# ksadov/FREUD

Hardware: AMD Instinct MI355X
Metric: SAE train activations/sec (d=384 dict 8x) (higher is better)
Workload: dtype bf16; 1 GPU; Whisper-tiny d=384 dict 8x (n=3072) L1 SAE train step, M=65536 rows/GPU/step, RAdam+cosine, x bfloat16 resident in HBM (BASELINE configs[1]); rows_per_gpu=65536, d_model=384, n_dict=3072, parallelism=dp1, dp=none

## Files before the change

freud_amd/csrc/bwd_fused.h:

```cpp
#pragma once
#include "common.h"
#include "gemm.h"

constexpr int BF_D = 384;
constexpr int BF_BM = 32;
constexpr int BF_BN = 128;
constexpr int BF_DXH_BYTES = BF_BM * BF_D * 2;
constexpr int BF_C_BYTES = BF_BM * BF_BN * 2;
constexpr int BF_STAGE_BYTES = 2 * BF_DXH_BYTES + BF_C_BYTES;
constexpr int BF_LDS_BYTES = 2 * BF_STAGE_BYTES;

__device__ __forceinline__ int dual_off(int row, int ch) {
  return row * 256 + ((ch ^ (((row & 3) << 2) | ((row >> 2) & 3))) << 4);
}

struct BwdFusedArgs {
  const bf16_t* dxh;
  const bf16_t* xb;
  const bf16_t* c;
  const bf16_t* Wt;
  const float* scal;
  int unscaled;
  const float* cnt_part;
  int n_cnt;
  float alpha;
  int64_t M;
  int d;
  float* slab;
  float* db_part;
  int n_p;
  int ntiles;
  int tile0;
  int splits;
  int steps_total;
  int bal_m, bal_q;
  const short* wg_map;
  unsigned long long* clk;
};

__device__ __forceinline__ bf16x8 tr_frag_perm(const char* img, int col0, int s, int lane) {
  const int h = lane >> 5, g = (lane >> 4) & 1, q = (lane & 15) >> 2, p = lane & 3;
  const int col = col0 + 16 * g + 4 * p;
  const int r0 = 16 * s + 4 * h + q, r1 = r0 + 8;
  const int o0 = dual_off(r0, col >> 3) + (col & 7) * 2;
  const int o1 = dual_off(r1, col >> 3) + (col & 7) * 2;
  const s16x4 lo = __builtin_amdgcn_ds_read_tr16_b64_v4i16(LDS_PTR(s16x4, img + o0));
  const s16x4 hi = __builtin_amdgcn_ds_read_tr16_b64_v4i16(LDS_PTR(s16x4, img + o1));
  typedef __attribute__((ext_vector_type(8))) short s16x8;
  const s16x8 v = __builtin_shufflevector(lo, hi, 0, 1, 2, 3, 4, 5, 6, 7);
  return __builtin_bit_cast(bf16x8, v);
}

constexpr int BF_RING = 12;

__device__ __forceinline__ void glds16_x2_add(const void* sbase0, const void* sbase1, unsigned voff0, unsigned voff1, unsigned base,
                                              unsigned l0, unsigned l1) {
  asm volatile(
      "s_add_u32 m0, %4, %5\n\ts_nop 0\n\tglobal_load_lds_dwordx4 %2, %0\n\t"
      "s_add_u32 m0, %4, %6\n\ts_nop 0\n\tglobal_load_lds_dwordx4 %3, %1"
      :
      : "s"(sbase0), "s"(sbase1), "v"(voff0), "v"(voff1), "s"(base), "s"(l0), "s"(l1)
      : "memory", "m0", "scc");
}
__device__ __forceinline__ void glds16_add(const void* sbase, unsigned voff, unsigned base, unsigned l0) {
  asm volatile("s_add_u32 m0, %2, %3\n\ts_nop 0\n\tglobal_load_lds_dwordx4 %1, %0" : : "s"(sbase), "v"(voff), "s"(base), "s"(l0) : "memory", "m0", "scc");
}
__device__ __forceinline__ void glds16_add_nt(const void* sbase, unsigned voff, unsigned base, unsigned l0) {
  asm volatile("s_add_u32 m0, %2, %3\n\ts_nop 0\n\tglobal_load_lds_dwordx4 %1, %0 nt" : : "s"(sbase), "v"(voff), "s"(base), "s"(l0) : "memory", "m0", "scc");
}
__device__ __forceinline__ void glds16_x2_add_nt(const void* sbase0, const void* sbase1, unsigned voff0, unsigned voff1, unsigned base,
                                                 unsigned l0, unsigned l1) {
  asm volatile(
      "s_add_u32 m0, %4, %5\n\ts_nop 0\n\tglobal_load_lds_dwordx4 %2, %0 nt\n\t"
      "s_add_u32 m0, %4, %6\n\ts_nop 0\n\tglobal_load_lds_dwordx4 %3, %1 nt"
      :
      : "s"(sbase0), "s"(sbase1), "v"(voff0), "v"(voff1), "s"(base), "s"(l0), "s"(l1)
      : "memory", "m0", "scc");
}

__global__ __launch_bounds__(256, 1) void bwd_fused_d384_kernel(BwdFusedArgs a) {
  extern __shared__ __attribute__((aligned(16))) char smem[];
  const int t = threadIdx.x, lane = t & 63, w = t >> 6;
  int qa = 0, qe = 1, wgk = 0;
  unsigned long long clk_k0 = 0;
  if (a.clk) clk_k0 = __builtin_amdgcn_s_memtime();
  int wgk_raw = (int)blockIdx.x;
  if (a.bal_m > 0 && a.wg_map) wgk_raw = (int)a.wg_map[blockIdx.x];
  double cnt_m = 0;
  if (a.cnt_part) {
    for (int i0 = t; i0 < a.n_cnt; i0 += 1024) {
      float cv[4];
#pragma unroll
      for (int u = 0; u < 4; ++u) cv[u] = a.cnt_part[min(i0 + 256 * u, a.n_cnt - 1)];
#pragma unroll
      for (int u = 0; u < 4; ++u) cnt_m += i0 + 256 * u < a.n_cnt ? (double)cv[u] : 0.0;
    }
  }
  if (a.bal_m > 0) {
    wgk = __builtin_amdgcn_readfirstlane(wgk_raw);
    qa = wgk * a.bal_m;
    qe = qa + a.bal_m < 32 * a.ntiles ? qa + a.bal_m : 32 * a.ntiles;
  }
  int n0 = 0, nw = 0;
  float scal1, scal2;
  if (a.cnt_part) {
    double* redc = reinterpret_cast<double*>(smem + BF_DXH_BYTES);
    double m = wave_sum_d(cnt_m);
    if (lane == 0) redc[w] = m;
    __syncthreads();
    const double count = (double)a.M * a.d - ((redc[0] + redc[1]) + (redc[2] + redc[3]));
    scal1 = a.alpha / (float)count;
    scal2 = 1.0f / (float)a.M;
    __syncthreads();
  } else {
    scal1 = a.scal[1];
    scal2 = a.scal[2];
  }
  const float scale = a.unscaled ? scal1 : 1.0f;
  const float inv_m = a.unscaled ? scal2 / scal1 : scal2;

  const int srow = lane >> 4;
  const int pc = lane & 15;
  unsigned voff_d[6], voff_c[2];
  unsigned loff_d[6];
#pragma unroll
// ... 72 lines not shown
  constexpr int RING = BF_RING, DIST = RING - 1;
  static_assert(72 % RING == 0, "ring slots must be static across steps");
  auto load_frag_s = [&](auto stage_tag, int i) -> bf16x8 {
    constexpr int ST = decltype(stage_tag)::value;
    if (i < 24) {
      return *reinterpret_cast<const bf16x8*>(smem + ST * BF_DXH_BYTES + (i >> 3) * 8192 + roff[i & 7]);
    } else {
      const int tt = i < 48 ? i - 24 : i - 48, dt = tt >> 1, sk = tt & 1;
      const char* b = smem + ST * BF_DXH_BYTES + (dt >> 2) * 8192 + sk * 4096;
      return i < 48 ? tr_pair(b + toff[2 * (dt & 3)], b + toff[2 * (dt & 3) + 1]) : tr_pair(b + toffX[2 * (dt & 3)], b + toffX[2 * (dt & 3) + 1]);
    }
  };
  auto load_c_s = [&](auto stage_tag, int half) -> bf16x8 {
    constexpr int ST = decltype(stage_tag)::value;
    const char* b = smem + ST * BF_C_BYTES + half * 4096;
    return tr_pair(b + coffC0, b + coffC1);
  };
  f32x16 cinit;
#pragma unroll
  for (int r = 0; r < 16; ++r) cinit[r] = inv_m;

  unsigned long long clk_t0 = 0, clk_r0 = 0, clk_loop = 0, clk_real = 0, clk_steps = 0;
#pragma unroll 1
  for (bool first_seg = true; qa < qe; first_seg = false) {
  bf16x8 wfrag[24];
  f32x16 acc[12];
  float db_acc = 0.f;
  bf16x8 ring[RING], cf[2], pf[2];
  int ntile, step_begin, step_end, split;
  if (a.bal_m > 0) {
    const int j = qa >> 5, qb = qe < 32 * (j + 1) ? qe : 32 * (j + 1);
    ntile = a.tile0 + j;
    step_begin = (qa - 32 * j) * a.bal_q;
    step_end = (qb - 32 * j) * a.bal_q;
    if (step_begin > a.steps_total) step_begin = a.steps_total;
    if (step_end > a.steps_total) step_end = a.steps_total;
    split = wgk - bal_first_wg(j, a.bal_m);
    qa = qb;
  } else {
    const int nblk = a.ntiles * a.splits;
    const int id = xcd_remap(blockIdx.x, nblk);
    split = id / a.ntiles;
    ntile = a.tile0 + id - split * a.ntiles;
    step_begin = (int)((int64_t)a.steps_total * split / a.splits);
    step_end = (int)((int64_t)a.steps_total * (split + 1) / a.splits);
    qa = qe;
  }
  ntile = __builtin_amdgcn_readfirstlane(ntile); step_begin = __builtin_amdgcn_readfirstlane(step_begin);
  step_end = __builtin_amdgcn_readfirstlane(step_end); split = __builtin_amdgcn_readfirstlane(split);
  n0 = ntile * BF_BN;
  nw = n0 + 32 * w;
  if (!first_seg) {
    asm volatile("s_waitcnt vmcnt(0) lgkmcnt(0)" ::: "memory");
    __syncthreads();
  }
  {
    const bf16_t* wp = a.Wt + (int64_t)(nw + (lane & 31)) * BF_D + 8 * (lane >> 5);
#pragma unroll
    for (int kk = 0; kk < 24; ++kk) wfrag[kk] = *reinterpret_cast<const bf16x8*>(wp + 16 * kk);
  }
#pragma unroll
  for (int i = 0; i < 12; ++i)
#pragma unroll
    for (int r = 0; r < 16; ++r) acc[i][r] = 0.f;
  db_acc = 0.f;
  if (step_begin < step_end) {
    const int64_t r0 = (int64_t)step_begin * BF_BM;
#pragma unroll
    for (int p = 0; p < 7; ++p) dma_pair_at(p, a.dxh + r0 * BF_D, a.xb + r0 * BF_D, a.c + r0 * a.n_p + n0, 0);
// ... 105 lines not shown
```

freud_amd/csrc/common.h:

```cpp
#pragma once
#include <hip/hip_runtime.h>
#include <stdint.h>

typedef __bf16 bf16_t;
typedef __attribute__((ext_vector_type(8))) __bf16 bf16x8;
typedef __attribute__((ext_vector_type(4))) __bf16 bf16x4;
typedef __attribute__((ext_vector_type(2))) __bf16 bf16x2;
typedef __attribute__((ext_vector_type(4))) short s16x4;
typedef __attribute__((ext_vector_type(16))) float f32x16;
typedef __attribute__((ext_vector_type(4))) float f32x4;
typedef __attribute__((ext_vector_type(4))) unsigned int u32x4;

#define LDS_PTR(T, p) ((__attribute__((address_space(3))) T*)(p))

__device__ __forceinline__ float bf16_round(float v) { return (float)(bf16_t)v; }

__device__ __forceinline__ float wave_sum(float v) {
#pragma unroll
  for (int o = 32; o > 0; o >>= 1) v += __shfl_xor(v, o, 64);
  return v;
}
__device__ __forceinline__ double wave_sum_d(double v) {
#pragma unroll
  for (int o = 32; o > 0; o >>= 1) v += __shfl_xor(v, o, 64);
// ... 44 lines not shown
      :
      : "s"(sbase0), "s"(sbase1), "v"(voff0), "v"(voff1), "s"(dst0), "s"(dst1)
      : "memory", "m0");
}

__device__ __forceinline__ void glds4(const void* sbase, unsigned voff, unsigned dst) {
  asm volatile("s_mov_b32 m0, %2\n\ts_nop 0\n\tglobal_load_lds_dword %1, %0" : : "s"(sbase), "v"(voff), "s"(dst) : "memory", "m0");
}

__device__ __forceinline__ void glds16(const void* sbase, unsigned voff, unsigned dst) {
  asm volatile("s_mov_b32 m0, %2\n\ts_nop 0\n\tglobal_load_lds_dwordx4 %1, %0" : : "s"(sbase), "v"(voff), "s"(dst) : "memory", "m0");
}

#include <type_traits>
template <int B, int E, class F>
__device__ __forceinline__ void static_for(F&& f) {
  if constexpr (B < E) {
    f(std::integral_constant<int, B>{});
    static_for<B + 1, E>(f);
  }
}

static inline int64_t round_up(int64_t v, int64_t m) { return (v + m - 1) / m * m; }

__host__ __device__ __forceinline__ int bal_first_wg(int j, int m) { return (32 * j) / m; }
__host__ __device__ __forceinline__ int bal_pieces(int j, int m) { return (32 * j + 31) / m - (32 * j) / m + 1; }
```

freud_amd/csrc/engine.hip:

```cpp
#include <hip/hip_runtime.h>
#include <math.h>
#include <stdarg.h>
#include <stdio.h>
#include <string.h>

#include <algorithm>
#include <utility>
#include <vector>

#include "../../include/freud_sae.h"
#include "l1_kernels.h"
#include "gemm256.h"
#include "gemm256s.h"
#include "gemm256_fp8.h"
#include "l1_fp8.h"
#include "dp_kernels.h"
#include "p2p_exchange.h"
#include <rccl/rccl.h>
#include <mutex>
#include <unistd.h>

static thread_local bool g_force_gemm128 = false;
static thread_local bool g_no_stream = false;
static thread_local int g_device = 0;
#include "bwd_fused.h"
#include "fwd_fused.h"
#include "fwd_fused2.h"
#include "topk_kernels.h"
#include "topk_sparse.h"
#include "topk_aux.h"
#include "eval_fp32.h"
#include "search.h"
#include "file_top.h"
#include "stats.h"
#include "coact.h"
#include "labels.h"
#include "manip.h"
#include "dict_match.h"

constexpr int G2_PERSIST_STATIC = 512;

static thread_local char g_err[512] = "";
static int fail(int code, const char* fmt, ...) {
  va_list ap;
  va_start(ap, fmt);
  vsnprintf(g_err, sizeof(g_err), fmt, ap);
  va_end(ap);
  return code;
// ... 187 lines not shown
  int dist_error = 0;
  char dist_errmsg[256] = "";
  bool p2p = false;
  int p2p_rank = 0;
  float* p2p_G[P2P_MAX_WORLD] = {};
  bf16_t* p2p_Gb[P2P_MAX_WORLD] = {};
  double* p2p_stats[P2P_MAX_WORLD] = {};
  unsigned long long* p2p_sig[P2P_MAX_WORLD] = {};
  void* p2p_opened[4 * P2P_MAX_WORLD] = {};
  int p2p_nopened = 0;
  unsigned long long* sig = nullptr;
  unsigned int* p2p_status = nullptr;
  unsigned int* p2p_status_host = nullptr;
  unsigned int* p2p_status_hostdev = nullptr;
  int p2p_fault_kind = 0, p2p_fault_rank = -1;
  unsigned long long p2p_fault_after = 0;
  float* col_stage = nullptr;
  float* audit_dst = nullptr;
  bool finegrained = false;
  unsigned long long p2p_epoch[P2P_CHANNELS] = {};
  unsigned long long p2p_epoch_push = 0;
  unsigned long long p2p_timeout_ticks = 12000000000ull;
  bool gn_from_exchange = false;
  int bal_m = 0;
  int bal_grid = 0;
  short* bal_map = nullptr;
  int bwd_ranges = 1;
  bool stats_inline = true;
  bool no_stream = false;
  int eval_prec = 0;
  LastCall last_call = LAST_FWD_BF16;
  void* fs_slab = nullptr;
  int8_t* co_zt = nullptr;
  int8_t* lb_lt = nullptr;
  int lb_rows = 0;
  float* mn_w = nullptr;
  int64_t e32_rows = 0;
  float *e32_x = nullptr, *e32_pre = nullptr, *e32_sel = nullptr, *e32_xhat = nullptr;
  double* e32_part = nullptr;
  int* e32_colmax = nullptr;
  int64_t step = 0;
  int64_t last_M = 0, last_M_p = 0;
  int last_dtype = 0;
  int profile = 0;
  int64_t prof_tick = 0;
  int prof_period = 8;
  EvRing ev[KID_COUNT];
  bool ev_init = false;
};
// ... 50 lines not shown
  }
}

extern "C" const char* sae_last_error(void) { return g_err; }
extern "C" int sae_version(void) { return 1; }
extern "C" const char* sae_kernel_name(int id) { return (id >= 0 && id < KID_COUNT) ? kKernelNames[id] : nullptr; }
extern "C" int sae_dominant_kernel(sae_ctx* c) { return c ? dominant_kid(c) : KID_DW; }

static int choose_splits(int r128, int c128, int64_t ktiles) {
  const bool big = !g_force_gemm128 && r128 % 2 == 0 && c128 % 2 == 0;
  const int tiles = big ? (r128 / 2) * (c128 / 2) : r128 * c128, slots = big ? 256 : 512;
  int best = 1;
  double best_cost = 1e30;
  for (int sp = 1; sp <= 16; ++sp) {
    if (sp > 1 && ktiles / sp < 8) break;
    const int rounds = (tiles * sp + slots - 1) / slots;
    const double cost = (double)rounds / sp + 0.04 * sp;
    if (cost < best_cost - 1e-9) {
      best_cost = cost;
      best = sp;
    }
  }
  return best;
}

static int fused_bwd_splits(int ntiles, int steps, int cols) {
  const double slab_steps = (double)cols * BF_D * 8.0 / 4.0e12 / 1.43e-6;
  int best = 1;
  double best_cost = 1e300;
  for (int sp = 1; sp <= 64 && sp <= steps; ++sp) {
    const int rounds = (ntiles * sp + 255) / 256;
    const double cost = rounds * ((double)((steps + sp - 1) / sp) + 5.0) + sp * slab_steps;
    if (cost < best_cost - 1e-9) {
      best_cost = cost;
      best = sp;
    }
  }
  return best;
}

static hipError_t peer_visible_malloc(const sae_ctx* c, void** p, size_t bytes) {
  if (c->finegrained) return hipExtMallocWithFlags(p, bytes, hipDeviceMallocFinegrained);
  return hipMalloc(p, bytes);
}

static int create_events(sae_ctx* c) {
// ... 120 lines not shown
  HIP_TRY(hipDeviceSynchronize());
  return SAE_OK;
}

extern "C" void sae_destroy(sae_ctx* c) {
  if (!c) return;
  (void)hipSetDevice(c->cfg.device_id);
  void* ptrs[] = {c->P,    c->Mom,     c->Var,     c->G,       c->Wb,   c->Wt,      c->xb,    c->c, c->dxh, c->dxhT, c->xT,
                  c->dpre, c->slab,    c->db_part, c->l1_part, c->sq_part, c->scal, c->gn_part, c->masked, c->cn_part, c->cnt_part,
                  c->We_b, c->Wd_b, c->xs, c->pre, c->dense, c->aux_dense, c->de_b, c->dh_b, c->e, c->dh, c->e2_part,
                  c->a2_part, c->dbd_part, c->ds_part, c->tkf, c->top_idx, c->aux_idx, c->tk, c->tv_part, c->nfsf, c->dead, c->dbe_fx,
                  c->multi_dense, c->multi_idx, c->em, c->dm_b, c->m2_part, c->x8, c->c8, c->W8, c->W8t, c->scal8, c->x8_part, c->dxh8,
                  c->stats, c->stats_part, c->Gb, c->top_vals, c->aux_vals, c->multi_vals, c->tile_max, c->sel_flag, c->csc_counts, c->csc_block_off, c->csc_total, c->csc_start, c->csc_item_start,
                  c->csc_item_latent, c->csc_entries, c->csc_part, c->csc_pbe, c->tkd, c->dead_cols, c->vec_rank, c->vec_bits, c->Wdd_b,
                  c->aux_dbe_part, c->be_r, c->cnorm, c->dw_tail, c->csc_multi, c->fs_slab, c->co_zt, c->lb_lt, c->mn_w};
  for (void* p : ptrs)
    if (p) (void)hipFree(p);
  if (c->dead_hint) (void)hipHostFree(c->dead_hint);
  for (int i = 0; i < c->p2p_nopened; ++i) (void)hipIpcCloseMemHandle(c->p2p_opened[i]);
  if (c->sig) (void)hipFree(c->sig);
  if (c->p2p_status) (void)hipFree(c->p2p_status);
  if (c->p2p_status_host) (void)hipHostFree(c->p2p_status_host);
  if (c->col_stage) (void)hipFree(c->col_stage);
  if (c->bal_map) (void)hipFree(c->bal_map);
  for (void* p : {(void*)c->e32_x, (void*)c->e32_pre, (void*)c->e32_sel, (void*)c->e32_xhat, (void*)c->e32_part, (void*)c->e32_colmax})
    if (p) (void)hipFree(p);
  if (c->comm) (void)ncclCommDestroy(c->comm);
  if (c->comm_stream) (void)hipStreamDestroy(c->comm_stream);
  for (hipEvent_t e : {c->ev_x, c->ev_stats, c->ev_done})
    if (e) (void)hipEventDestroy(e);
  for (hipEvent_t e : c->ev_range)
    if (e) (void)hipEventDestroy(e);
  if (c->ev_init)
    for (auto& r : c->ev)
      for (int i = 0; i < EV_RING; ++i) {
        if (r.beg[i]) (void)hipEventDestroy(r.beg[i]);
        if (r.end[i]) (void)hipEventDestroy(r.end[i]);
      }
  delete c;
}

extern "C" int sae_create(const sae_config* cfg, sae_ctx** out) {
  if (!cfg || !out) return fail(SAE_ERR_INVALID, "null argument");
  *out = nullptr;
  if (cfg->variant != SAE_VARIANT_L1 && cfg->variant != SAE_VARIANT_TOPK)
    return fail(SAE_ERR_INVALID, "Invalid autoencoder variant: %d, must be 'l1' or 'topk'", cfg->variant);
  if (cfg->variant == SAE_VARIANT_TOPK && (cfg->k <= 0 || cfg->k > cfg->n_dict || cfg->k > 1024))
// ... 57 lines not shown
    gemm_tail_plan((c->d_p / 256) * (c->n_p / 256), (int)(2 * Mp / 64), c->dw_tail_tiles, c->dw_tail_pieces);
    if ((c->d_p / 256) * (c->n_p / 256) % 256 == 0) c->dw_tail_tiles = c->dw_tail_pieces = -1;
  }
  c->dw_chunk_splits = choose_splits(c->dw_chunk_rows / 128, c->n_p / 128, 2 * Mp / 64);
  if (c->d_p >= 1024 && c->n_p % 256 == 0)
    for (int q = 4; q >= 2; --q)
      if ((c->n_p / 256) % q == 0) {
        c->dw_col_chunks = q;
        break;
      }
  c->dw_col_splits = choose_splits(c->d_p / 128, c->n_p / 128 / c->dw_col_chunks, 2 * Mp / 64);
  c->use_fused_bwd = (c->d_p == BF_D) && cfg->force_generic != 1 && !c->fp8;
  c->use_fused_fwd = (c->d_p == FF_D) && cfg->force_generic != 1 && !c->fp8;
  if (const char* fv = getenv("FREUD_FWD")) c->fwd_variant = atoi(fv) == 1 ? 1 : 2;
  c->bwd_splits = fused_bwd_splits(c->n_p / BF_BN, (int)(Mp / BF_BM), c->n_p);
  c->bwd_range_splits = c->bwd_splits;
  for (int r = 2; r <= 4; ++r)
    if ((c->n_p / BF_BN) % r == 0) {
      const int sp = fused_bwd_splits(c->n_p / BF_BN / r, (int)(Mp / BF_BM), c->n_p / r);
      if (sp > c->bwd_range_splits) c->bwd_range_splits = sp;
    }
  int slab_splits = c->use_fused_bwd ? (c->bwd_range_splits > c->dw_splits ? c->bwd_range_splits : c->dw_splits) : c->dw_splits;
  if (c->use_fused_bwd && c->cfg.debug_flags != 83 && !getenv("FREUD_BWD_UNIFORM")) {
    const int ntiles = c->n_p / BF_BN, cus = 256;
    const int m = (32 * ntiles + cus - 1) / cus, grid = (32 * ntiles + m - 1) / m;
    int pmax = 1;
    for (int j = 0; j < ntiles; ++j) pmax = bal_pieces(j, m) > pmax ? bal_pieces(j, m) : pmax;
    const int steps = (int)(Mp / BF_BM), q = (steps + 31) / 32;
    const double slab_steps = (double)c->n_p * BF_D * 8.0 / 4.0e12 / 1.43e-6;
    const double cost_bal = (double)m * q + 5.0 + (32 % m ? 3.5 : 0.0) + (32.0 / m + (32 % m ? 1.0 : 0.0)) * slab_steps;
    const int sp = c->bwd_splits, rounds = (ntiles * sp + 255) / 256;
    const double cost_uni = rounds * ((double)((steps + sp - 1) / sp) + 5.0) + sp * slab_steps;
    if (cost_bal < cost_uni * 0.995 && pmax <= 64 && grid <= 4096) {
      c->bal_m = m;
      c->bal_grid = grid;
      if (pmax > slab_splits) slab_splits = pmax;
      std::vector<int> order(grid);
      for (int k = 0; k < grid; ++k) order[k] = k;
      std::stable_sort(order.begin(), order.end(), [m](int a_, int b_) { return (a_ * m) % 32 < (b_ * m) % 32; });
      std::vector<short> map(grid);
      int pos = 0;
      for (int x = 0; x < 8; ++x) {
        const int len = grid / 8 + (x < grid % 8 ? 1 : 0);
        for (int i = 0; i < len; ++i) map[8 * i + x] = (short)order[pos++];
      }
      hipError_t e_ = hipMalloc((void**)&c->bal_map, (size_t)grid * 2);
      if (e_ == hipSuccess) e_ = hipMemcpy(c->bal_map, map.data(), (size_t)grid * 2, hipMemcpyHostToDevice);
      if (e_ != hipSuccess) {
        int rc_ = fail(SAE_ERR_HIP, "balanced backward: workgroup table: %s", hipGetErrorString(e_));
        sae_destroy(c);
        return rc_;
      }
    }
  }
  {
    const int64_t need = (int64_t)(c->dw_chunk_splits > c->dw_col_splits ? c->dw_chunk_splits : c->dw_col_splits);
    if (need > slab_splits) slab_splits = (int)need;
  }
  const int64_t db_rows = (Mp / 128) > 64 ? (Mp / 128) : 64;

#define ALLOC(ptr, bytes)                                   \
  do {                                                      \
    hipError_t e_ = hipMalloc((void**)&(ptr), (bytes));     \
    if (e_ != hipSuccess) {                                 \
      int rc_ = fail(SAE_ERR_HIP, "hipMalloc(%lld bytes) for %s failed: %s", (long long)(bytes), #ptr, \
                     hipGetErrorString(e_));                \
      sae_destroy(c);                                       \
      return rc_;                                           \
    }                                                       \
  } while (0)
  ALLOC(c->P, c->nparams * 4);
  ALLOC(c->Mom, c->nparams * 4);
  ALLOC(c->Var, c->nparams * 4);
  if (c->finegrained) {
    hipError_t e_ = peer_visible_malloc(c, (void**)&c->G, (size_t)(c->nparams + SAE_NUM_METRICS) * 4);
    if (e_ == hipSuccess) e_ = peer_visible_malloc(c, (void**)&c->stats, (size_t)DP_STATS_HEAD * 8);
    if (e_ != hipSuccess) {
      int rc_ = fail(SAE_ERR_HIP, "fine-grained allocation of the gradient / statistics buffers failed: %s", hipGetErrorString(e_));
      sae_destroy(c);
      return rc_;
    }
  } else {
// ... 1009 lines not shown
  if (rc) return rc;
  const bool fold_finalize = c->use_fused_fwd && c->use_fused_bwd && backward && gs == nullptr && c->bwd_ranges == 1 &&
                             c->cfg.debug_flags != 78;
  if (c->use_fused_fwd && !fold_finalize) {
    StatsPush push{};
    if (gs && inline_stats(c)) {
      for (int r = 0; r < c->dp_world; ++r) push.inbox[r] = c->p2p_sig[r] + P2P_SIG_WORDS;
      push.rank = c->p2p_rank; push.world = c->dp_world; push.epoch = ++c->p2p_epoch_push;
      push.timeout_ticks = c->p2p_timeout_ticks; push.status = c->p2p_status; push.status_host = c->p2p_status_hostdev; push.gstats_out = c->stats;
    } else if (gs && c->dist) {
      HIP_TRY(hipStreamWaitEvent(s, c->ev_stats, 0));
    }
    if (push.world > 0) ev_begin(c, KID_STATS_XCHG, s);
    hipLaunchKernelGGL(finalize_losses_kernel, dim3(1), dim3(1024), 0, s, c->l1_part, (int)(Mp / 128), c->sq_part,
                       (int)(Mp / 128), c->scal, c->G + c->nparams, M, d, alpha, c->cnt_part, (int)(Mp / 128),
                       push.world > 0 ? (const double*)nullptr : gs, push);
    if (push.world > 0) ev_end(c, KID_STATS_XCHG, s);
  }
  bool dw_chunked_any = false;
  if (backward) {
    int splits = c->dw_splits;
    int db_rows = (int)(Mp / 128);
    bool dw_chunked = false;
    if (c->use_fused_bwd) {
      BwdFusedArgs a{};
      a.dxh = c->dxh; a.xb = c->xb_cur; a.c = c->c; a.Wt = c->Wt; a.scal = c->scal; a.slab = c->slab; a.db_part = c->db_part;
      a.unscaled = c->use_fused_fwd ? 1 : 0;
      if (fold_finalize) { a.cnt_part = c->cnt_part; a.n_cnt = (int)(Mp / 128); a.alpha = alpha; a.M = M; a.d = d; }
      a.n_p = n_p; a.steps_total = (int)(Mp / BF_BM);
      a.clk = c->cfg.debug_flags == 66 ? reinterpret_cast<unsigned long long*>(c->dpre) + (1 << 16) : nullptr;
      const int nranges = c->bwd_ranges, rtiles = (n_p / BF_BN) / nranges;
      splits = nranges == 1 ? c->bwd_splits : c->bwd_range_splits;
      if (splits > a.steps_total) splits = a.steps_total;
      a.ntiles = rtiles; a.splits = splits;
      db_rows = splits;
      const bool balanced = nranges == 1 && c->bal_m > 0 && a.steps_total >= 64;
      if (balanced) {
        a.bal_m = c->bal_m;
        a.bal_q = (a.steps_total + 31) / 32;
        a.wg_map = c->bal_map;
      }
      const bool dp_now = c->dist && c->dp_world > 0;
      bf16_t* gb = (dp_now && c->payload == SAE_DTYPE_BF16) ? c->Gb : (bf16_t*)nullptr;
      ev_begin(c, KID_BWD_FUSED, s);
      LDS_ATTR(bwd_fused_d384_kernel, BF_LDS_BYTES, g_device);
      for (int r = 0; r < nranges; ++r) {
        a.tile0 = r * rtiles;
        hipLaunchKernelGGL(bwd_fused_d384_kernel, dim3(balanced ? c->bal_grid : a.ntiles * a.splits), dim3(256), BF_LDS_BYTES, s, a);
        if (nranges > 1) {
          const int c0 = a.tile0 * BF_BN, cols = rtiles * BF_BN;
          hipLaunchKernelGGL(reduce_grads_range_kernel, dim3(256), dim3(256), 0, s, c->slab, c->nW, splits, c->db_part, db_rows, n_p,
                             d_p, c0, cols, c->G, c->gn_part + 256 * r, gb);
          if (dp_now && r + 1 < nranges) fused_exchange(c, r, nranges, c0, cols, false, s);
        }
      }
      ev_end(c, KID_BWD_FUSED, s);
      HIP_TRY(hipGetLastError());
    } else {
      if (c->fp8_bwd) {
        const int sgrid = (int)((Mp / 4) < 1024 ? (Mp / 4) : 1024);
        hipLaunchKernelGGL(fp8_x_stats_kernel, dim3(sgrid), dim3(256), 0, s, c->dxh, Mp, d_p, c->x8_part);
        hipLaunchKernelGGL(fp8_g_scale_kernel, dim3(1), dim3(256), 0, s, c->x8_part, sgrid, c->scal8);
        const int64_t n8 = Mp * (d_p / 8);
        hipLaunchKernelGGL(fp8_quant_x_kernel, dim3(grid_for(n8, 2048)), dim3(256), 0, s, c->dxh, c->dxh8, n8, c->scal8, (int)S8_SG);
        Gemm8Args g{};
        g.A = c->dxh8; g.B = c->W8t; g.lda = d_p; g.ldb = d_p;
        g.nbm = (int)(Mp / 256); g.nbn = n_p / 256; g.ktiles = d_p / 128;
        EpiDpre8 e{};
        e.c = c->c; e.dpre = c->dpre; e.db_part = c->db_part; e.scal = c->scal; e.scal8 = c->scal8; e.n_p = n_p;
        ev_begin(c, KID_DPRE, s);
        rc = launch_gemm8(g, e, s);
// ... 113 lines not shown
        }
      }
      if (!col_chunked) {
        ev_end(c, KID_DW, s);
        dw_chunked_any = chunked;
        dw_chunked = chunked || direct;
      }
    }
    ev_begin(c, KID_REDUCE, s);
    if (c->use_fused_bwd && c->bwd_ranges > 1) {
      c->gn_blocks = 256 * c->bwd_ranges;
      c->gn_valid = true;
    } else if (c->use_fused_bwd) {
      const int64_t nW4 = c->nW / 4, n4 = c->nparams / 4;
      const int blocks = grid_for(n4, 1024);
      LossFinalize fin{};
      if (fold_finalize) {
        fin.l1_part = c->l1_part; fin.sq_part = c->sq_part; fin.cnt_part = c->cnt_part; fin.n_parts = (int)(Mp / 128);
        fin.scal = c->scal; fin.metrics = c->G + c->nparams; fin.M = M; fin.d = d; fin.alpha = alpha;
      }
      hipLaunchKernelGGL(reduce_grads_kernel, dim3(blocks), dim3(256), 0, s, c->slab, nW4, splits, c->db_part, db_rows, n_p,
                         c->G, nW4, n4, c->gn_part,
                         (c->dist && c->dp_world > 0 && c->payload == SAE_DTYPE_BF16) ? c->Gb : (bf16_t*)nullptr, fin,
                         (c->bwd_ranges == 1 && c->bal_m > 0 && (int)(Mp / BF_BM) >= 64) ? c->bal_m : 0);
      c->gn_blocks = blocks;
      c->gn_valid = true;
    } else {
      const int64_t n4 = c->nW / 4;
      if (!dw_chunked)
        hipLaunchKernelGGL(reduce_slabs_kernel, dim3((unsigned)((n4 + 255) / 256)), dim3(256), 0, s, c->slab, c->G, n4, n4,
                           splits);
      hipLaunchKernelGGL(reduce_db_kernel, dim3(n_p / 32), dim3(256), 0, s, c->db_part, c->G + c->nW, db_rows, n_p);
      c->gn_valid = false;
    }
    ev_end(c, KID_REDUCE, s);
  }
  if (!c->use_fused_fwd)
    hipLaunchKernelGGL(finalize_losses_kernel, dim3(1), dim3(1024), 0, s, c->l1_part, (int)((Mp / 128) * (n_p / 128)),
                       c->sq_part, (int)((Mp / 128) * (d_p / 128)), c->scal, c->G + c->nparams, M, d, alpha,
                       (const float*)nullptr, 0, gs, StatsPush{});
  if (backward) {
    const int64_t total = c->nparams + SAE_NUM_METRICS;
    if (c->use_fused_bwd && c->dist && c->dp_world > 0) {
      const int nr = c->bwd_ranges, cols = n_p / nr;
      fused_exchange(c, nr - 1, nr, (nr - 1) * cols, cols, true, s);
    } else if (dw_chunked_any) notify_grads(c, c->nW, total - c->nW, s);
    else notify_grads(c, 0, total, s);
// ... 673 lines not shown
    return SAE_OK;
  }
  if (which >= 7 && which <= 9) {
    if (!c->fp8) return fail(SAE_ERR_INVALID, "not an fp8 context");
    if (which == 7) {
      if (cap < S8_COUNT) return fail(SAE_ERR_INVALID, "capacity too small");
      HIP_TRY(hipMemcpy(out, c->scal8, S8_COUNT * 4, hipMemcpyDeviceToHost));
      return SAE_OK;
    }
    const int cols = which == 8 ? c->d : c->n, ld = which == 8 ? c->d_p : c->n_p;
    if (cap < M * cols) return fail(SAE_ERR_INVALID, "capacity too small");
    std::vector<unsigned char> tmp((size_t)M * ld);
    HIP_TRY(hipMemcpy(tmp.data(), which == 8 ? c->x8 : c->c8, tmp.size(), hipMemcpyDeviceToHost));
    for (int64_t r = 0; r < M; ++r)
      for (int j = 0; j < cols; ++j) {
        const unsigned b = tmp[(size_t)r * ld + j], e = (b >> 3) & 15, m = b & 7;
        float v = e == 0 ? ldexpf((float)m, -9) : ldexpf(1.0f + m / 8.0f, (int)e - 7);
        if (e == 15 && m == 7) v = NAN;
        out[r * cols + j] = (b & 0x80) ? -v : v;
      }
    return SAE_OK;
  }
  if (which == 6) {
    const int64_t grid = (c->bal_m > 0 && c->bwd_ranges == 1) ? c->bal_grid : (int64_t)(c->n_p / 128) * c->bwd_splits;
    const int64_t nq = grid * 4 * 2;
    if (cap < nq) return fail(SAE_ERR_INVALID, "capacity too small");
    std::vector<unsigned long long> tmp((size_t)nq);
    HIP_TRY(hipMemcpy(tmp.data(), reinterpret_cast<unsigned long long*>(c->dpre) + (1 << 16), tmp.size() * 8, hipMemcpyDeviceToHost));
    for (int64_t i = 0; i < nq; ++i) out[i] = (float)tmp[(size_t)i];
    return SAE_OK;
  }
#ifdef CSCF_STAMP
  if (which == 13) {
    const int64_t rows = cap / 8 < 4096 ? cap / 8 : 4096;
    std::vector<unsigned long long> tmp((size_t)rows * 8);
    HIP_TRY(hipMemcpyFromSymbol(tmp.data(), HIP_SYMBOL(cscf_stamp_buf), tmp.size() * 8, 0, hipMemcpyDeviceToHost));
    for (int64_t i = 0; i < rows * 8; ++i) out[i] = (float)tmp[(size_t)i];
    return SAE_OK;
  }
#endif
#ifdef TSEL_STAMP
  if (which == 12) {
    const int64_t rows = cap / 8 < 4096 ? cap / 8 : 4096;
    std::vector<unsigned long long> tmp((size_t)rows * 8);
    HIP_TRY(hipMemcpyFromSymbol(tmp.data(), HIP_SYMBOL(tsel_stamp_buf), tmp.size() * 8, 0, hipMemcpyDeviceToHost));
    for (int64_t i = 0; i < rows * 8; ++i) out[i] = (float)tmp[(size_t)i];
    return SAE_OK;
// ... 779 lines not shown
```

freud_amd/csrc/l1_kernels.h:

```cpp
#pragma once
#include "gemm.h"

__device__ __forceinline__ float colnorm_tree8(const float (*red)[128], int col) {
  return ((red[0][col] + red[1][col]) + (red[2][col] + red[3][col])) + ((red[4][col] + red[5][col]) + (red[6][col] + red[7][col]));
}

__global__ __launch_bounds__(256) void colnorm_partial_kernel(const float* __restrict__ W, float* __restrict__ part,
                                                               int n_p) {
  __shared__ float red[8][128];
  const int t = threadIdx.x, tx = t & 31, ty = t >> 5;
  const int col = blockIdx.x * 128 + 4 * tx, r0 = blockIdx.y * 32;
  f32x4 ss = {0.f, 0.f, 0.f, 0.f};
#pragma unroll
  for (int i = 0; i < 4; ++i) {
    const f32x4 v = *reinterpret_cast<const f32x4*>(W + (int64_t)(r0 + ty + 8 * i) * n_p + col);
#pragma unroll
    for (int q = 0; q < 4; ++q) ss[q] = __builtin_fmaf(v[q], v[q], ss[q]);
  }
#pragma unroll
  for (int q = 0; q < 4; ++q) red[ty][4 * tx + q] = ss[q];
  __syncthreads();
  if (t < 128) part[(int64_t)blockIdx.y * n_p + blockIdx.x * 128 + t] = colnorm_tree8(red, t);
}

// ... 429 lines not shown
  __syncthreads();
  if (threadIdx.x == 0) {
    const double l1 = (redf[0][0] + redf[0][1]) + (redf[0][2] + redf[0][3]), sq = (redf[1][0] + redf[1][1]) + (redf[1][2] + redf[1][3]);
    const double pl = (redf[2][0] + redf[2][1]) + (redf[2][2] + redf[2][3]), masked = (redf[3][0] + redf[3][1]) + (redf[3][2] + redf[3][3]);
    const double local = (double)f.M * f.d - masked;
    f.scal[0] = (float)local;
    f.scal[1] = f.alpha / (float)local;
    f.scal[2] = 1.0f / (float)f.M;
    f.scal[3] = (float)local;
    const double count = (double)f.scal[0];
    f.metrics[0] = (float)((double)f.alpha * (sq / count));
    f.metrics[1] = (float)(l1 / (double)f.M);
    f.metrics[2] = (float)(pl / ((double)f.M * f.d));
    f.metrics[3] = 0.f;
    f.metrics[4] = f.scal[0];
    f.metrics[5] = f.metrics[6] = f.metrics[7] = 0.f;
  }
}

__global__ __launch_bounds__(256) void reduce_grads_kernel(const float* __restrict__ slab, int64_t stride4, int splits,
                                                            const float* __restrict__ db_part, int db_rows, int n_p,
                                                            float* __restrict__ grad, int64_t nW4, int64_t n4,
                                                            double* __restrict__ gn_part, bf16_t* __restrict__ grad_bf16,
                                                            LossFinalize fin, int bal_m) {
  __shared__ double red[4];
  if (fin.cnt_part && blockIdx.x == gridDim.x - 1) finalize_losses_block256(fin);
  double ss = 0;
  const int n4p = n_p / 4;
  auto add_pieces = [](f32x4 a, const f32x4* p, int64_t stride, int cnt) -> f32x4 {
    int k = 1;
    for (; k + 7 < cnt; k += 8) {
      f32x4 v[8];
#pragma unroll
      for (int u = 0; u < 8; ++u) v[u] = p[(k + u) * stride];
#pragma unroll
      for (int u = 0; u < 8; ++u) a += v[u];
    }
    if (k + 3 < cnt) {
      f32x4 v[4];
#pragma unroll
      for (int u = 0; u < 4; ++u) v[u] = p[(k + u) * stride];
#pragma unroll
      for (int u = 0; u < 4; ++u) a += v[u];
      k += 4;
    }
    if (k + 1 < cnt) {
      const f32x4 v0 = p[k * stride], v1 = p[(k + 1) * stride];
      a += v0;
      a += v1;
      k += 2;
    }
    if (k < cnt) a += p[k * stride];
    return a;
  };
  for (int64_t i = (int64_t)blockIdx.x * 256 + threadIdx.x; i < n4; i += (int64_t)gridDim.x * 256) {
    f32x4 a;
    if (i < nW4) {
      const f32x4* s = reinterpret_cast<const f32x4*>(slab);
      const int cnt = bal_m > 0 ? bal_pieces((int)(i % n4p) >> 5, bal_m) : splits;
      a = add_pieces(s[i], s + i, stride4, cnt);
    } else {
      const int64_t j4 = i - nW4;
      const f32x4* s = reinterpret_cast<const f32x4*>(db_part);
      const int cnt = bal_m > 0 ? bal_pieces((int)j4 >> 5, bal_m) : db_rows;
      a = add_pieces(s[j4], s + j4, (int64_t)n4p, cnt);
    }
    reinterpret_cast<f32x4*>(grad)[i] = a;
    if (grad_bf16) reinterpret_cast<bf16x4*>(grad_bf16)[i] = bf16x4{(bf16_t)a[0], (bf16_t)a[1], (bf16_t)a[2], (bf16_t)a[3]};
    ss += (double)(a[0] * a[0]) + (double)(a[1] * a[1]) + (double)(a[2] * a[2]) + (double)(a[3] * a[3]);
  }
  ss = wave_sum_d(ss);
  if ((threadIdx.x & 63) == 0) red[threadIdx.x >> 6] = ss;
  __syncthreads();
  if (threadIdx.x == 0) gn_part[blockIdx.x] = red[0] + red[1] + red[2] + red[3];
}

__global__ __launch_bounds__(256) void gnorm_from_bf16_kernel(const bf16_t* __restrict__ gb, float* __restrict__ grad, int64_t n4,
                                                               float scale, double* __restrict__ part) {
  __shared__ double red[4];
  double s = 0;
  for (int64_t i = (int64_t)blockIdx.x * 256 + threadIdx.x; i < n4; i += (int64_t)gridDim.x * 256) {
    const bf16x4 v = reinterpret_cast<const bf16x4*>(gb)[i];
    const f32x4 g = {(float)v[0], (float)v[1], (float)v[2], (float)v[3]};
    reinterpret_cast<f32x4*>(grad)[i] = g;
    const f32x4 q = g * scale;
    s += (double)(q[0] * q[0]) + (double)(q[1] * q[1]) + (double)(q[2] * q[2]) + (double)(q[3] * q[3]);
  }
// ... 492 lines not shown
```

Baseline: 119.7 million activations/s.

## Replace fixed balanced backward split with host-computed per-workgroup segment table

Swaps the closed-form balanced work split (bal_m, bal_q, wg_map) for a host-side partitioner that bisects a per-workgroup cost target, including a per-segment overhead, and emits up to two (tile, step range, piece) segments per workgroup. The kernel reads its segments from a device table, and reduce_grads reads per-tile piece counts from a device array. The aim is to even out load across the 256 CUs when tiles and steps do not divide nicely, cutting tail imbalance. It adds a table lookup per launch and host setup work, and changes how many slab pieces the gradient reduction sums.

```diff
diff --git a/freud_amd/csrc/bwd_fused.h b/freud_amd/csrc/bwd_fused.h
--- a/freud_amd/csrc/bwd_fused.h
+++ b/freud_amd/csrc/bwd_fused.h
@@ -33,8 +33,7 @@
   int tile0;
   int splits;
   int steps_total;
-  int bal_m, bal_q;
-  const short* wg_map;
+  const int4* seg_tab;
   unsigned long long* clk;
 };
 
@@ -81,11 +80,14 @@
 __global__ __launch_bounds__(256, 1) void bwd_fused_d384_kernel(BwdFusedArgs a) {
   extern __shared__ __attribute__((aligned(16))) char smem[];
   const int t = threadIdx.x, lane = t & 63, w = t >> 6;
-  int qa = 0, qe = 1, wgk = 0;
+  int seg_i = 0, seg_n = 1;
   unsigned long long clk_k0 = 0;
   if (a.clk) clk_k0 = __builtin_amdgcn_s_memtime();
-  int wgk_raw = (int)blockIdx.x;
-  if (a.bal_m > 0 && a.wg_map) wgk_raw = (int)a.wg_map[blockIdx.x];
+  int4 seg0 = {0, 0, 0, 0}, seg1 = {0, 0, 0, 0};
+  if (a.seg_tab) {
+    seg0 = a.seg_tab[2 * blockIdx.x];
+    seg1 = a.seg_tab[2 * blockIdx.x + 1];
+  }
   double cnt_m = 0;
   if (a.cnt_part) {
     for (int i0 = t; i0 < a.n_cnt; i0 += 1024) {
@@ -96,11 +98,7 @@
       for (int u = 0; u < 4; ++u) cnt_m += i0 + 256 * u < a.n_cnt ? (double)cv[u] : 0.0;
     }
   }
-  if (a.bal_m > 0) {
-    wgk = __builtin_amdgcn_readfirstlane(wgk_raw);
-    qa = wgk * a.bal_m;
-    qe = qa + a.bal_m < 32 * a.ntiles ? qa + a.bal_m : 32 * a.ntiles;
-  }
+  if (a.seg_tab) seg_n = __builtin_amdgcn_readfirstlane(seg1.z > seg1.y ? 2 : 1);
   int n0 = 0, nw = 0;
   float scal1, scal2;
   if (a.cnt_part) {
@@ -219,21 +217,18 @@
 
   unsigned long long clk_t0 = 0, clk_r0 = 0, clk_loop = 0, clk_real = 0, clk_steps = 0;
 #pragma unroll 1
-  for (bool first_seg = true; qa < qe; first_seg = false) {
+  for (bool first_seg = true; seg_i < seg_n; first_seg = false, ++seg_i) {
   bf16x8 wfrag[24];
   f32x16 acc[12];
   float db_acc = 0.f;
   bf16x8 ring[RING], cf[2], pf[2];
   int ntile, step_begin, step_end, split;
-  if (a.bal_m > 0) {
-    const int j = qa >> 5, qb = qe < 32 * (j + 1) ? qe : 32 * (j + 1);
-    ntile = a.tile0 + j;
-    step_begin = (qa - 32 * j) * a.bal_q;
-    step_end = (qb - 32 * j) * a.bal_q;
-    if (step_begin > a.steps_total) step_begin = a.steps_total;
-    if (step_end > a.steps_total) step_end = a.steps_total;
-    split = wgk - bal_first_wg(j, a.bal_m);
-    qa = qb;
+  if (a.seg_tab) {
+    const int4 sg = seg_i ? seg1 : seg0;
+    ntile = a.tile0 + sg.x;
+    step_begin = sg.y;
+    step_end = sg.z;
+    split = sg.w;
   } else {
     const int nblk = a.ntiles * a.splits;
     const int id = xcd_remap(blockIdx.x, nblk);
@@ -241,7 +236,6 @@
     ntile = a.tile0 + id - split * a.ntiles;
     step_begin = (int)((int64_t)a.steps_total * split / a.splits);
     step_end = (int)((int64_t)a.steps_total * (split + 1) / a.splits);
-    qa = qe;
   }
   ntile = __builtin_amdgcn_readfirstlane(ntile); step_begin = __builtin_amdgcn_readfirstlane(step_begin);
   step_end = __builtin_amdgcn_readfirstlane(step_end); split = __builtin_amdgcn_readfirstlane(split);
diff --git a/freud_amd/csrc/bwd_partition.h b/freud_amd/csrc/bwd_partition.h
--- /dev/null
+++ b/freud_amd/csrc/bwd_partition.h
@@ -0,0 +1,189 @@
+#pragma once
+#include <algorithm>
+#include <vector>
+
+constexpr double BWD_SEG_OVERHEAD_STEPS = 8.4;
+constexpr int BWD_MAX_PIECES = 64;
+
+struct BwdSeg {
+  int tile, step_begin, step_end, piece;
+};
+struct BwdWg {
+  int nseg;
+  BwdSeg seg[2];
+};
+struct BwdPartition {
+  std::vector<BwdWg> wg;
+  std::vector<int> pieces;
+  int pmax = 0;
+  double max_cost = 0, min_cost = 0;
+};
+
+static inline int bwd_gcd(int a, int b) {
+  while (b) {
+    const int t = a % b;
+    a = b;
+    b = t;
+  }
+  return a;
+}
+
+static inline double bwd_wg_cost(const BwdWg& w, double o) {
+  double c = 0;
+  for (int s = 0; s < w.nseg; ++s) c += (double)(w.seg[s].step_end - w.seg[s].step_begin) + o;
+  return c;
+}
+
+static inline double bwd_spread(const std::vector<BwdWg>& wg, double o) {
+  double mx = 0, mn = 1e300;
+  for (const BwdWg& w : wg) {
+    const double c = bwd_wg_cost(w, o);
+    mx = std::max(mx, c);
+    mn = std::min(mn, c);
+  }
+  return mx - mn;
+}
+
+static inline int bwd_fill(int P, int S, double o, double T_hi, int a_hi, int limit, std::vector<BwdWg>* out) {
+  int tile = 0, step = 0, n = 0;
+  if (out) out->clear();
+  while (tile < P) {
+    if (n > limit) return n;
+    const double T = n < a_hi ? T_hi : T_hi - 1.0;
+    BwdWg w{};
+    int take = (int)(T - o);
+    if (take < 1) take = 1;
+    if (take > S - step) take = S - step;
+    w.nseg = 1;
+    w.seg[0] = BwdSeg{tile, step, step + take, 0};
+    step += take;
+    if (step == S) {
+      ++tile;
+      step = 0;
+      if (tile < P) {
+        int room = (int)(T_hi - (double)take - 2.0 * o);
+        const int room_own = (int)(T - (double)take - 2.0 * o);
+        if (room >= 1 && room_own < 1) room = 1;
+        else room = room_own;
+        if (room >= 1) {
+          if (room > S) room = S;
+          w.nseg = 2;
+          w.seg[1] = BwdSeg{tile, 0, room, 0};
+          step = room;
+          if (step == S) {
+            ++tile;
+            step = 0;
+          }
+        }
+      }
+    }
+    if (out) out->push_back(w);
+    ++n;
+  }
+  return n;
+}
+
+static inline void bwd_level(std::vector<BwdWg>& wg, int P) {
+  size_t i = 0;
+  while (i < wg.size()) {
+    if (wg[i].nseg != 1) {
+      ++i;
+      continue;
+    }
+    size_t e = i;
+    while (e < wg.size() && wg[e].nseg == 1 && wg[e].seg[0].tile == wg[i].seg[0].tile) ++e;
+    const int n = (int)(e - i), b0 = wg[i].seg[0].step_begin, total = wg[e - 1].seg[0].step_end - b0;
+    int b = b0;
+    for (int k = 0; k < n; ++k) {
+      const int take = total / n + (k < total % n ? 1 : 0);
+      wg[i + k].seg[0].step_begin = b;
+      wg[i + k].seg[0].step_end = b + take;
+      b += take;
+    }
+    i = e;
+  }
+  (void)P;
+}
+
+static inline std::vector<BwdWg> bwd_pattern(int P, int S, int K, double o) {
+  double lo = 1.0 + o, hi = (double)P * S + 2.0 * o + 1.0;
+  if (bwd_fill(P, S, o, lo, K, K, nullptr) <= K) hi = lo;
+  else if (bwd_fill(P, S, o, hi, K, K, nullptr) > K) {
+    return std::vector<BwdWg>();
+  } else {
+    for (int it = 0; it < 64 && hi - lo > 1e-6; ++it) {
+      const double mid = 0.5 * (lo + hi);
+      if (bwd_fill(P, S, o, mid, K, K, nullptr) <= K) hi = mid;
+      else lo = mid;
+    }
+  }
+  const double T = hi;
+  std::vector<BwdWg> pat, alt;
+  bwd_fill(P, S, o, T, K, K, &pat);
+  bwd_level(pat, P);
+  double best = bwd_spread(pat, o);
+  if (T - 1.0 - o >= 1.0)
+    for (int a = K - 1; a >= 0 && best > 1.0 + o; --a) {
+      if (bwd_fill(P, S, o, T, a, K, &alt) > K) continue;
+      bwd_level(alt, P);
+      const double sp = bwd_spread(alt, o);
+      if (sp < best) {
+        best = sp;
+        pat.swap(alt);
+      }
+    }
+  return pat;
+}
+
+static inline BwdPartition bwd_partition(int ntiles, int steps_total, int cus, double o) {
+  BwdPartition part;
+  if (ntiles < 1 || steps_total < 1 || cus < 1) return part;
+  const int g = bwd_gcd(ntiles, cus), P = ntiles / g, S = steps_total;
+  std::vector<BwdWg> pat;
+  for (int K = cus / g; K >= 1;) {
+    pat = bwd_pattern(P, S, K, o);
+    if (pat.empty()) return part;
+    std::vector<int> cnt(P, 0);
+    int pm = 0;
+    for (const BwdWg& w : pat)
+      for (int s = 0; s < w.nseg; ++s) pm = std::max(pm, ++cnt[w.seg[s].tile]);
+    if (pm <= BWD_MAX_PIECES) break;
+    K = std::min(K - 1, (int)((long long)K * BWD_MAX_PIECES / pm));
+    pat.clear();
+  }
+  if (pat.empty()) return part;
+  part.pieces.assign(ntiles, 0);
+  part.wg.reserve(pat.size() * g);
+  for (int r = 0; r < g; ++r)
+    for (const BwdWg& w0 : pat) {
+      BwdWg w = w0;
+      for (int s = 0; s < w.nseg; ++s) {
+        w.seg[s].tile += r * P;
+        w.seg[s].piece = part.pieces[w.seg[s].tile]++;
+      }
+      part.wg.push_back(w);
+    }
+  part.max_cost = 0;
+  part.min_cost = 1e300;
+  for (const BwdWg& w : part.wg) {
+    const double c = bwd_wg_cost(w, o);
+    part.max_cost = std::max(part.max_cost, c);
+    part.min_cost = std::min(part.min_cost, c);
+  }
+  for (int p : part.pieces) part.pmax = std::max(part.pmax, p);
+  return part;
+}
+
+static inline std::vector<int> bwd_wg_order(const BwdPartition& part) {
+  const int n = (int)part.wg.size();
+  std::vector<int> order(n), map(n);
+  for (int k = 0; k < n; ++k) order[k] = k;
+  std::stable_sort(order.begin(), order.end(),
+                   [&part](int a, int b) { return part.wg[a].seg[0].step_begin < part.wg[b].seg[0].step_begin; });
+  int pos = 0;
+  for (int x = 0; x < 8; ++x) {
+    const int len = n / 8 + (x < n % 8 ? 1 : 0);
+    for (int i = 0; i < len; ++i) map[8 * i + x] = order[pos++];
+  }
+  return map;
+}
diff --git a/freud_amd/csrc/common.h b/freud_amd/csrc/common.h
--- a/freud_amd/csrc/common.h
+++ b/freud_amd/csrc/common.h
@@ -90,6 +90,3 @@
 }
 
 static inline int64_t round_up(int64_t v, int64_t m) { return (v + m - 1) / m * m; }
-
-__host__ __device__ __forceinline__ int bal_first_wg(int j, int m) { return (32 * j) / m; }
-__host__ __device__ __forceinline__ int bal_pieces(int j, int m) { return (32 * j + 31) / m - (32 * j) / m + 1; }
diff --git a/freud_amd/csrc/engine.hip b/freud_amd/csrc/engine.hip
--- a/freud_amd/csrc/engine.hip
+++ b/freud_amd/csrc/engine.hip
@@ -24,6 +24,7 @@
 static thread_local bool g_no_stream = false;
 static thread_local int g_device = 0;
 #include "bwd_fused.h"
+#include "bwd_partition.h"
 #include "fwd_fused.h"
 #include "fwd_fused2.h"
 #include "topk_kernels.h"
@@ -257,9 +258,15 @@
   unsigned long long p2p_epoch_push = 0;
   unsigned long long p2p_timeout_ticks = 12000000000ull;
   bool gn_from_exchange = false;
-  int bal_m = 0;
+  struct BalTable {
+    int steps = 0, grid = 0, pmax = 0;
+    int4* segs = nullptr;
+    int* pieces = nullptr;
+  };
+  bool bal_on = false;
   int bal_grid = 0;
-  short* bal_map = nullptr;
+  int bal_slab_cap = 0;
+  std::vector<BalTable> bal_tabs;
   int bwd_ranges = 1;
   bool stats_inline = true;
   bool no_stream = false;
@@ -356,6 +363,42 @@
     }
   }
   return best;
+}
+
+constexpr int BAL_CUS = 256;
+
+static const sae_ctx::BalTable* bal_table_for(sae_ctx* c, int steps, int& rc) {
+  rc = SAE_OK;
+  for (const auto& t : c->bal_tabs)
+    if (t.steps == steps) return t.grid > 0 ? &t : nullptr;
+  sae_ctx::BalTable t;
+  t.steps = steps;
+  const int ntiles = c->n_p / BF_BN;
+  const BwdPartition part = bwd_partition(ntiles, steps, BAL_CUS, BWD_SEG_OVERHEAD_STEPS);
+  if (!part.wg.empty() && part.pmax <= c->bal_slab_cap && part.pmax <= BWD_MAX_PIECES) {
+    const int grid = (int)part.wg.size();
+    const std::vector<int> order = bwd_wg_order(part);
+    std::vector<int4> segs((size_t)2 * grid);
+    for (int b = 0; b < grid; ++b) {
+      const BwdWg& w = part.wg[order[b]];
+      segs[2 * b] = int4{w.seg[0].tile, w.seg[0].step_begin, w.seg[0].step_end, w.seg[0].piece};
+      segs[2 * b + 1] = w.nseg == 2 ? int4{w.seg[1].tile, w.seg[1].step_begin, w.seg[1].step_end, w.seg[1].piece} : int4{0, 0, 0, 0};
+    }
+    hipError_t e = hipMalloc((void**)&t.segs, segs.size() * sizeof(int4));
+    if (e == hipSuccess) e = hipMalloc((void**)&t.pieces, (size_t)ntiles * sizeof(int));
+    if (e == hipSuccess) e = hipMemcpy(t.segs, segs.data(), segs.size() * sizeof(int4), hipMemcpyHostToDevice);
+    if (e == hipSuccess) e = hipMemcpy(t.pieces, part.pieces.data(), (size_t)ntiles * sizeof(int), hipMemcpyHostToDevice);
+    if (e != hipSuccess) {
+      if (t.segs) (void)hipFree(t.segs);
+      if (t.pieces) (void)hipFree(t.pieces);
+      rc = fail(SAE_ERR_HIP, "balanced backward: segment table for %d steps: %s", steps, hipGetErrorString(e));
+      return nullptr;
+    }
+    t.grid = grid;
+    t.pmax = part.pmax;
+  }
+  c->bal_tabs.push_back(t);
+  return t.grid > 0 ? &c->bal_tabs.back() : nullptr;
 }
 
 static int fused_bwd_splits(int ntiles, int steps, int cols) {
@@ -522,7 +565,11 @@
   if (c->p2p_status) (void)hipFree(c->p2p_status);
   if (c->p2p_status_host) (void)hipHostFree(c->p2p_status_host);
   if (c->col_stage) (void)hipFree(c->col_stage);
-  if (c->bal_map) (void)hipFree(c->bal_map);
+  for (auto& t : c->bal_tabs) {
+    if (t.segs) (void)hipFree(t.segs);
+    if (t.pieces) (void)hipFree(t.pieces);
+  }
+  c->bal_tabs.clear();
   for (void* p : {(void*)c->e32_x, (void*)c->e32_pre, (void*)c->e32_sel, (void*)c->e32_xhat, (void*)c->e32_part, (void*)c->e32_colmax})
     if (p) (void)hipFree(p);
   if (c->comm) (void)ncclCommDestroy(c->comm);
@@ -626,35 +673,15 @@
     }
   int slab_splits = c->use_fused_bwd ? (c->bwd_range_splits > c->dw_splits ? c->bwd_range_splits : c->dw_splits) : c->dw_splits;
   if (c->use_fused_bwd && c->cfg.debug_flags != 83 && !getenv("FREUD_BWD_UNIFORM")) {
-    const int ntiles = c->n_p / BF_BN, cus = 256;
-    const int m = (32 * ntiles + cus - 1) / cus, grid = (32 * ntiles + m - 1) / m;
-    int pmax = 1;
-    for (int j = 0; j < ntiles; ++j) pmax = bal_pieces(j, m) > pmax ? bal_pieces(j, m) : pmax;
-    const int steps = (int)(Mp / BF_BM), q = (steps + 31) / 32;
+    const int ntiles = c->n_p / BF_BN, steps = (int)(Mp / BF_BM);
+    const BwdPartition part = bwd_partition(ntiles, steps, BAL_CUS, BWD_SEG_OVERHEAD_STEPS);
     const double slab_steps = (double)c->n_p * BF_D * 8.0 / 4.0e12 / 1.43e-6;
-    const double cost_bal = (double)m * q + 5.0 + (32 % m ? 3.5 : 0.0) + (32.0 / m + (32 % m ? 1.0 : 0.0)) * slab_steps;
+    const double cost_bal = part.max_cost + part.pmax * slab_steps;
     const int sp = c->bwd_splits, rounds = (ntiles * sp + 255) / 256;
-    const double cost_uni = rounds * ((double)((steps + sp - 1) / sp) + 5.0) + sp * slab_steps;
-    if (cost_bal < cost_uni * 0.995 && pmax <= 64 && grid <= 4096) {
-      c->bal_m = m;
-      c->bal_grid = grid;
-      if (pmax > slab_splits) slab_splits = pmax;
-      std::vector<int> order(grid);
-      for (int k = 0; k < grid; ++k) order[k] = k;
-      std::stable_sort(order.begin(), order.end(), [m](int a_, int b_) { return (a_ * m) % 32 < (b_ * m) % 32; });
-      std::vector<short> map(grid);
-      int pos = 0;
-      for (int x = 0; x < 8; ++x) {
-        const int len = grid / 8 + (x < grid % 8 ? 1 : 0);
-        for (int i = 0; i < len; ++i) map[8 * i + x] = (short)order[pos++];
-      }
-      hipError_t e_ = hipMalloc((void**)&c->bal_map, (size_t)grid * 2);
-      if (e_ == hipSuccess) e_ = hipMemcpy(c->bal_map, map.data(), (size_t)grid * 2, hipMemcpyHostToDevice);
-      if (e_ != hipSuccess) {
-        int rc_ = fail(SAE_ERR_HIP, "balanced backward: workgroup table: %s", hipGetErrorString(e_));
-        sae_destroy(c);
-        return rc_;
-      }
+    const double cost_uni = rounds * ((double)((steps + sp - 1) / sp) + BWD_SEG_OVERHEAD_STEPS) + sp * slab_steps;
+    if (!part.wg.empty() && (cost_bal < cost_uni * 0.995 || getenv("FREUD_BWD_BALANCED"))) {
+      c->bal_on = true;
+      if (part.pmax > slab_splits) slab_splits = part.pmax;
     }
   }
   {
@@ -662,6 +689,15 @@
     if (need > slab_splits) slab_splits = (int)need;
   }
   const int64_t db_rows = (Mp / 128) > 64 ? (Mp / 128) : 64;
+  c->bal_slab_cap = slab_splits;
+  if (c->bal_on && Mp / BF_BM >= 64) {
+    int rc_ = SAE_OK;
+    (void)bal_table_for(c, (int)(Mp / BF_BM), rc_);
+    if (rc_) {
+      sae_destroy(c);
+      return rc_;
+    }
+  }
 
 #define ALLOC(ptr, bytes)                                   \
   do {                                                      \
@@ -1717,6 +1753,7 @@
     int splits = c->dw_splits;
     int db_rows = (int)(Mp / 128);
     bool dw_chunked = false;
+    const int* bal_pieces_dev = nullptr;
     if (c->use_fused_bwd) {
       BwdFusedArgs a{};
       a.dxh = c->dxh; a.xb = c->xb_cur; a.c = c->c; a.Wt = c->Wt; a.scal = c->scal; a.slab = c->slab; a.db_part = c->db_part;
@@ -1729,11 +1766,17 @@
       if (splits > a.steps_total) splits = a.steps_total;
       a.ntiles = rtiles; a.splits = splits;
       db_rows = splits;
-      const bool balanced = nranges == 1 && c->bal_m > 0 && a.steps_total >= 64;
+      const sae_ctx::BalTable* bal = nullptr;
+      if (nranges == 1 && c->bal_on && a.steps_total >= 64) {
+        int rc_tab = SAE_OK;
+        bal = bal_table_for(c, a.steps_total, rc_tab);
+        if (rc_tab) return rc_tab;
+      }
+      const bool balanced = bal != nullptr;
       if (balanced) {
-        a.bal_m = c->bal_m;
-        a.bal_q = (a.steps_total + 31) / 32;
-        a.wg_map = c->bal_map;
+        a.seg_tab = bal->segs;
+        bal_pieces_dev = bal->pieces;
+        c->bal_grid = bal->grid;
       }
       const bool dp_now = c->dist && c->dp_world > 0;
       bf16_t* gb = (dp_now && c->payload == SAE_DTYPE_BF16) ? c->Gb : (bf16_t*)nullptr;
@@ -1741,7 +1784,7 @@
       LDS_ATTR(bwd_fused_d384_kernel, BF_LDS_BYTES, g_device);
       for (int r = 0; r < nranges; ++r) {
         a.tile0 = r * rtiles;
-        hipLaunchKernelGGL(bwd_fused_d384_kernel, dim3(balanced ? c->bal_grid : a.ntiles * a.splits), dim3(256), BF_LDS_BYTES, s, a);
+        hipLaunchKernelGGL(bwd_fused_d384_kernel, dim3(balanced ? bal->grid : a.ntiles * a.splits), dim3(256), BF_LDS_BYTES, s, a);
         if (nranges > 1) {
           const int c0 = a.tile0 * BF_BN, cols = rtiles * BF_BN;
           hipLaunchKernelGGL(reduce_grads_range_kernel, dim3(256), dim3(256), 0, s, c->slab, c->nW, splits, c->db_part, db_rows, n_p,
@@ -1901,7 +1944,7 @@
       hipLaunchKernelGGL(reduce_grads_kernel, dim3(blocks), dim3(256), 0, s, c->slab, nW4, splits, c->db_part, db_rows, n_p,
                          c->G, nW4, n4, c->gn_part,
                          (c->dist && c->dp_world > 0 && c->payload == SAE_DTYPE_BF16) ? c->Gb : (bf16_t*)nullptr, fin,
-                         (c->bwd_ranges == 1 && c->bal_m > 0 && (int)(Mp / BF_BM) >= 64) ? c->bal_m : 0);
+                         bal_pieces_dev);
       c->gn_blocks = blocks;
       c->gn_valid = true;
     } else {
@@ -2621,7 +2664,7 @@
     return SAE_OK;
   }
   if (which == 6) {
-    const int64_t grid = (c->bal_m > 0 && c->bwd_ranges == 1) ? c->bal_grid : (int64_t)(c->n_p / 128) * c->bwd_splits;
+    const int64_t grid = (c->bal_on && c->bwd_ranges == 1 && c->bal_grid > 0) ? c->bal_grid : (int64_t)(c->n_p / 128) * c->bwd_splits;
     const int64_t nq = grid * 4 * 2;
     if (cap < nq) return fail(SAE_ERR_INVALID, "capacity too small");
     std::vector<unsigned long long> tmp((size_t)nq);
diff --git a/freud_amd/csrc/l1_kernels.h b/freud_amd/csrc/l1_kernels.h
--- a/freud_amd/csrc/l1_kernels.h
+++ b/freud_amd/csrc/l1_kernels.h
@@ -475,7 +475,7 @@
                                                             const float* __restrict__ db_part, int db_rows, int n_p,
                                                             float* __restrict__ grad, int64_t nW4, int64_t n4,
                                                             double* __restrict__ gn_part, bf16_t* __restrict__ grad_bf16,
-                                                            LossFinalize fin, int bal_m) {
+                                                            LossFinalize fin, const int* __restrict__ tile_pieces) {
   __shared__ double red[4];
   if (fin.cnt_part && blockIdx.x == gridDim.x - 1) finalize_losses_block256(fin);
   double ss = 0;
@@ -510,12 +510,12 @@
     f32x4 a;
     if (i < nW4) {
       const f32x4* s = reinterpret_cast<const f32x4*>(slab);
-      const int cnt = bal_m > 0 ? bal_pieces((int)(i % n4p) >> 5, bal_m) : splits;
+      const int cnt = tile_pieces ? tile_pieces[(int)(i % n4p) >> 5] : splits;
       a = add_pieces(s[i], s + i, stride4, cnt);
     } else {
       const int64_t j4 = i - nW4;
       const f32x4* s = reinterpret_cast<const f32x4*>(db_part);
-      const int cnt = bal_m > 0 ? bal_pieces((int)j4 >> 5, bal_m) : db_rows;
+      const int cnt = tile_pieces ? tile_pieces[(int)j4 >> 5] : db_rows;
       a = add_pieces(s[j4], s + j4, (int64_t)n4p, cnt);
     }
     reinterpret_cast<f32x4*>(grad)[i] = a;
```

Result: no change. 120.7 million activations/s (median of 6 runs) (+0.8%).
